# ermongroup/TEOChat

Hardware: AMD Instinct MI355X
Metric: end-to-end tokens/sec (prefill+decode), T=8 frames, LLaMA-2-7B (higher is better)
Workload: dtype bf16; 1 GPU; C3: T=8 frames 224x224 -> CLIP-ViT-L/14 (23 layers) -> mlp2x_gelu -> splice of a 128-token prompt (L=2168) -> LLaMA-2-7B prefill -> 256 forced greedy tokens; value = generated tokens / total time; frames=8, sequence_len=2168, parallelism=dp1 (1 conversation per GPU, no collective), weights=random N(0,0.02^2) at LLaMA-2-7B / ViT-L/14 shapes

## Files before the change

teochat_amd/csrc/gemv.hip:

```cpp
#include <type_traits>

#include "ops.h"
#include "p13.h"

namespace teo {

typedef unsigned char fp8_t;
typedef float f32x2 __attribute__((ext_vector_type(2)));

template <typename T> struct Vec16;
template <> struct Vec16<bf16_t> {
    static constexpr int N = 8;
    __device__ static __forceinline__ void cvt(const uint4& r, float* f) {
        f[0] = __uint_as_float(r.x << 16); f[1] = __uint_as_float(r.x & 0xffff0000u);
        f[2] = __uint_as_float(r.y << 16); f[3] = __uint_as_float(r.y & 0xffff0000u);
        f[4] = __uint_as_float(r.z << 16); f[5] = __uint_as_float(r.z & 0xffff0000u);
        f[6] = __uint_as_float(r.w << 16); f[7] = __uint_as_float(r.w & 0xffff0000u);
    }
};
template <> struct Vec16<f16_t> {
    static constexpr int N = 8;
    __device__ static __forceinline__ void cvt(const uint4& r, float* f) {
        f[0] = h_lo<true>(r.x); f[1] = h_hi<true>(r.x); f[2] = h_lo<true>(r.y); f[3] = h_hi<true>(r.y);
        f[4] = h_lo<true>(r.z); f[5] = h_hi<true>(r.z); f[6] = h_lo<true>(r.w); f[7] = h_hi<true>(r.w);
    }
};
template <> struct Vec16<float> {
    static constexpr int N = 4;
    __device__ static __forceinline__ void cvt(const uint4& r, float* f) {
        f[0] = __uint_as_float(r.x); f[1] = __uint_as_float(r.y); f[2] = __uint_as_float(r.z); f[3] = __uint_as_float(r.w);
    }
};
struct fp4x2_t { unsigned char v; };
template <typename WT> struct IsMx { static constexpr bool v = false; };
template <> struct IsMx<fp4x2_t> { static constexpr bool v = true; };
template <> struct Vec16<fp4x2_t> { static constexpr int N = 32; };
template <typename WT> struct WPer { static constexpr int v = IsMx<WT>::v ? 2 : 1; };
template <typename WT> struct CU { static constexpr int v = Vec16<WT>::N / WPer<WT>::v; };
template <typename WT> using WScaleT = typename std::conditional<IsMx<WT>::v, unsigned char, float>::type;
template <> struct Vec16<fp8_t> {
    static constexpr int N = 16;
    __device__ static __forceinline__ void cvt(const uint4& r, float* f) {
        const unsigned w[4] = {r.x, r.y, r.z, r.w};
#pragma unroll
        for (int i = 0; i < 4; ++i) {
            const f32x2 lo = __builtin_amdgcn_cvt_pk_f32_fp8(w[i], false);
            const f32x2 hi = __builtin_amdgcn_cvt_pk_f32_fp8(w[i], true);
            f[4 * i] = lo.x; f[4 * i + 1] = lo.y; f[4 * i + 2] = hi.x; f[4 * i + 3] = hi.y;
        }
    }
};

template <typename WT>
__device__ __forceinline__ float dot16(const uint4& w, const float* xv, float acc) {
    constexpr int VE = Vec16<WT>::N;
    float f[VE];
    Vec16<WT>::cvt(w, f);
#pragma unroll
    for (int e = 0; e < VE; ++e) acc = fmaf(f[e], xv[e], acc);
    return acc;
}
template <>
__device__ __forceinline__ float dot16<fp8_t>(const uint4& w, const float* xv, float acc) {
    const unsigned ww[4] = {w.x, w.y, w.z, w.w};
#pragma unroll
    for (int i = 0; i < 4; ++i) {
        const f32x2 lo = __builtin_amdgcn_cvt_pk_f32_fp8(ww[i], false);
        const f32x2 hi = __builtin_amdgcn_cvt_pk_f32_fp8(ww[i], true);
        acc = fmaf(lo.x, xv[4 * i], acc);
        acc = fmaf(lo.y, xv[4 * i + 1], acc);
        acc = fmaf(hi.x, xv[4 * i + 2], acc);
        acc = fmaf(hi.y, xv[4 * i + 3], acc);
    }
    return acc;
}

typedef __bf16 gv_bf16x2 __attribute__((ext_vector_type(2)));
__device__ __forceinline__ float dot2bf(unsigned a, unsigned b, float acc) {
    return __builtin_amdgcn_fdot2_f32_bf16(__builtin_bit_cast(gv_bf16x2, a), __builtin_bit_cast(gv_bf16x2, b), acc, false);
}
template <typename WT>
__device__ __forceinline__ float dotb(const uint4& w, const uint4* xv, float acc) {
    constexpr bool F16 = IsF16<WT>::v;
    acc = dot2h<F16>(w.x, xv[0].x, acc); acc = dot2h<F16>(w.y, xv[0].y, acc);
    acc = dot2h<F16>(w.z, xv[0].z, acc); acc = dot2h<F16>(w.w, xv[0].w, acc);
    return acc;
}
template <>
__device__ __forceinline__ float dotb<fp8_t>(const uint4& w, const uint4* xv, float acc) {
    const unsigned ww[4] = {w.x, w.y, w.z, w.w};
    const unsigned xx[8] = {xv[0].x, xv[0].y, xv[0].z, xv[0].w, xv[1].x, xv[1].y, xv[1].z, xv[1].w};
#pragma unroll
    for (int i = 0; i < 4; ++i) {
        const unsigned lo = __builtin_bit_cast(unsigned, __builtin_amdgcn_cvt_scalef32_pk_bf16_fp8(ww[i], 1.0f, false));
        const unsigned hi = __builtin_bit_cast(unsigned, __builtin_amdgcn_cvt_scalef32_pk_bf16_fp8(ww[i], 1.0f, true));
        acc = dot2bf(lo, xx[2 * i], acc);
        acc = dot2bf(hi, xx[2 * i + 1], acc);
    }
    return acc;
}
__device__ __forceinline__ float dot_mx(const uint4& w, const uint4* xv, float escale, float acc) {
    const unsigned ww[4] = {w.x, w.y, w.z, w.w};
#pragma unroll
    for (int i = 0; i < 4; ++i) {
        acc = dot2bf(__builtin_bit_cast(unsigned, __builtin_amdgcn_cvt_scalef32_pk_bf16_fp4(ww[i], escale, 0)), xv[i].x, acc);
        acc = dot2bf(__builtin_bit_cast(unsigned, __builtin_amdgcn_cvt_scalef32_pk_bf16_fp4(ww[i], escale, 1)), xv[i].y, acc);
        acc = dot2bf(__builtin_bit_cast(unsigned, __builtin_amdgcn_cvt_scalef32_pk_bf16_fp4(ww[i], escale, 2)), xv[i].z, acc);
        acc = dot2bf(__builtin_bit_cast(unsigned, __builtin_amdgcn_cvt_scalef32_pk_bf16_fp4(ww[i], escale, 3)), xv[i].w, acc);
    }
    return acc;
}
__device__ __forceinline__ float e8m0_scale(unsigned e) { return __uint_as_float(e << 23); }
template <typename T> struct IsBf { static constexpr bool v = false; };
template <> struct IsBf<bf16_t> { static constexpr bool v = true; };
template <typename T> struct Is16 { static constexpr bool v = IsBf<T>::v || IsF16<T>::v; };
template <typename T, typename WT> struct BfImage { static constexpr bool v = IsBf<T>::v && sizeof(WT) == 1; };
template <typename T, typename WT> struct RowsImage16 { static constexpr bool v = BfImage<T, WT>::v || (IsF16<T>::v && IsF16<WT>::v); };

struct p13_t { unsigned short v; };
template <typename WT> struct IsP13 { static constexpr bool v = false; };
template <> struct IsP13<p13_t> { static constexpr bool v = true; };
template <> struct Vec16<p13_t> {
    static constexpr int N = 8;
    __device__ static __forceinline__ void cvt(const uint4& r, float* f) {
#pragma unroll
        for (int i = 0; i < 4; ++i) { f[i] = __uint_as_float(p13_f32(r.z, r.x, i)); f[4 + i] = __uint_as_float(p13_f32(r.w, r.y, i)); }
    }
};
struct P13Img {
    const unsigned* rt; const unsigned char *lo, *nib, *sgn; const bf16_t* esc;
};
__device__ __forceinline__ P13Img p13_img(const void* W, int N, int K) {
    const P13Layout l = p13_layout(N, K);
    const unsigned char* b = reinterpret_cast<const unsigned char*>(W);
    return {reinterpret_cast<const unsigned*>(b + l.rt), b + l.lo, b + l.nib, b + l.sgn, reinterpret_cast<const bf16_t*>(b + l.esc)};
}
template <bool NT, typename V>
__device__ __forceinline__ V ldv(const void* p) {
    return NT ? __builtin_nontemporal_load(reinterpret_cast<const V*>(p)) : *reinterpret_cast<const V*>(p);
}
template <bool NT>
__device__ __forceinline__ uint4 p13_load(const unsigned char* lo, const unsigned char* nib, const unsigned char* sgn, long long c) {
    typedef unsigned v2u __attribute__((ext_vector_type(2)));
    const v2u l = ldv<NT, v2u>(lo + c * 8);
    return make_uint4(l.x, l.y, ldv<NT, unsigned>(nib + c * 4), (unsigned)ldv<NT, unsigned char>(sgn + c));
}
template <bool PAIRS>
__device__ __forceinline__ uint4 p13_chunk(const uint4& raw, unsigned rpm) {
    if constexpr (PAIRS) {
        unsigned o[4];
        p13_rebuild(raw.x, raw.y, raw.z, raw.w, rpm, o);
        return make_uint4(o[0], o[1], o[2], o[3]);
    } else {
        unsigned h0, h1;
        p13_high(raw.z, raw.w, rpm, h0, h1);
        return make_uint4(raw.x, raw.y, h0, h1);
    }
}
__device__ __forceinline__ unsigned p13_rpm(unsigned rt) { return ((rt & 0xffu) - 1u) * 0x00010001u; }
__device__ __forceinline__ bool p13_escaped(unsigned rt) { return (rt & 0xffu) == 0xffu; }

template <bool NT>
__device__ __forceinline__ uint4 ld16(const void* p) {
    typedef unsigned v4u __attribute__((ext_vector_type(4)));
    const v4u v = NT ? __builtin_nontemporal_load(reinterpret_cast<const v4u*>(p)) : *reinterpret_cast<const v4u*>(p);
    return make_uint4(v.x, v.y, v.z, v.w);
}


template <int VE>
__device__ __forceinline__ int xs_off(int k) {
    const int c = k / VE, g = (k % VE) >> 2;
    return (((c >> 6) * (VE / 4) + g) << 8) + ((c & 63) << 2);
}
template <int VE>
__device__ __forceinline__ int xb_off(int k) {
    const int c = k / VE, g = (k % VE) >> 3;
    return ((((c >> 6) * (VE / 8) + g) << 6) + (c & 63)) * 8 + (k & 7);
}
template <bool XB, int VE>
__device__ __forceinline__ float* x_image_end(float* xs, int nchunk) {
    const int padded = ((nchunk + 63) / 64) * 64 * VE;
    return XB ? reinterpret_cast<float*>(reinterpret_cast<bf16_t*>(xs) + padded) : xs + padded;
}

template <typename T, int VE, bool XB, int XPT, typename F>
__device__ __forceinline__ void stage_x(const T* __restrict__ x, const T* __restrict__ norm_w, float* xs, float* red, int K,
                                        float eps, F after_loads) {
    constexpr int VX = Vec16<T>::N;
    const int tid = threadIdx.x;
    const int nx = K / VX;
    float ss = 0.f;
    if (nx <= XPT * GV_THREADS) {
        uint4 xr[XPT], nr[XPT];
#pragma unroll
        for (int i = 0; i < XPT; ++i) {
            const int c = tid + i * GV_THREADS;
            xr[i] = (c < nx) ? *reinterpret_cast<const uint4*>(x + (long long)c * VX) : make_uint4(0, 0, 0, 0);
        }
        if (norm_w) {
#pragma unroll
            for (int i = 0; i < XPT; ++i) {
                const int c = tid + i * GV_THREADS;
                nr[i] = (c < nx) ? *reinterpret_cast<const uint4*>(norm_w + (long long)c * VX) : make_uint4(0, 0, 0, 0);
            }
        }
        after_loads();
#pragma unroll
        for (int i = 0; i < XPT; ++i) {
            float f[VX];
            Vec16<T>::cvt(xr[i], f);
#pragma unroll
            for (int e = 0; e < VX; ++e) ss = fmaf(f[e], f[e], ss);
        }
        float rr = 1.f;
        if (norm_w) rr = rsqrtf(block_sum<GV_THREADS>(ss, red) / K + eps);
#pragma unroll
        for (int i = 0; i < XPT; ++i) {
            const int c = tid + i * GV_THREADS;
            if (c < nx) {
                float f[VX], g[VX];
                Vec16<T>::cvt(xr[i], f);
                if (norm_w) {
                    Vec16<T>::cvt(nr[i], g);
#pragma unroll
                    for (int e = 0; e < VX; ++e) f[e] = Elem<T>::round(f[e] * rr * g[e]);
                }
                if constexpr (XB) {
                    uint4 o = xr[i];
                    if (norm_w) o = make_uint4(pack_h2<IsF16<T>::v>(f[0], f[1]), pack_h2<IsF16<T>::v>(f[2], f[3]), pack_h2<IsF16<T>::v>(f[4], f[5]),
                                               pack_h2<IsF16<T>::v>(f[6], f[7]));
                    *reinterpret_cast<uint4*>(reinterpret_cast<bf16_t*>(xs) + xb_off<VE>(c * VX)) = o;
                } else {
#pragma unroll
                    for (int e = 0; e < VX; e += 4)
                        *reinterpret_cast<float4*>(xs + xs_off<VE>(c * VX + e)) = make_float4(f[e], f[e + 1], f[e + 2], f[e + 3]);
                }
            }
        }
    } else {
        after_loads();
        for (int c = tid; c < nx; c += GV_THREADS) {
            const uint4 raw = *reinterpret_cast<const uint4*>(x + (long long)c * VX);
            float f[VX];
            Vec16<T>::cvt(raw, f);
#pragma unroll
            for (int e = 0; e < VX; ++e) ss = fmaf(f[e], f[e], ss);
            if constexpr (XB) {
                *reinterpret_cast<uint4*>(reinterpret_cast<bf16_t*>(xs) + xb_off<VE>(c * VX)) = raw;
            } else {
#pragma unroll
                for (int e = 0; e < VX; e += 4)
                    *reinterpret_cast<float4*>(xs + xs_off<VE>(c * VX + e)) = make_float4(f[e], f[e + 1], f[e + 2], f[e + 3]);
            }
        }
        if (norm_w) {
            const float rr = rsqrtf(block_sum<GV_THREADS>(ss, red) / K + eps);
            for (int c = tid; c < nx; c += GV_THREADS) {
                float f[VX];
                Vec16<T>::cvt(*reinterpret_cast<const uint4*>(norm_w + (long long)c * VX), f);
                if constexpr (XB) {
                    uint4* p4 = reinterpret_cast<uint4*>(reinterpret_cast<bf16_t*>(xs) + xb_off<VE>(c * VX));
                    float v[VX];
                    Vec16<T>::cvt(*p4, v);
#pragma unroll
                    for (int e = 0; e < VX; ++e) v[e] = v[e] * rr * f[e];
                    *p4 = make_uint4(pack_h2<IsF16<T>::v>(v[0], v[1]), pack_h2<IsF16<T>::v>(v[2], v[3]), pack_h2<IsF16<T>::v>(v[4], v[5]),
                                     pack_h2<IsF16<T>::v>(v[6], v[7]));
                } else {
#pragma unroll
                    for (int e = 0; e < VX; e += 4) {
                        float4* p4 = reinterpret_cast<float4*>(xs + xs_off<VE>(c * VX + e));
                        float4 v = *p4;
                        v.x = Elem<T>::round(v.x * rr * f[e]); v.y = Elem<T>::round(v.y * rr * f[e + 1]);
                        v.z = Elem<T>::round(v.z * rr * f[e + 2]); v.w = Elem<T>::round(v.w * rr * f[e + 3]);
                        *p4 = v;
                    }
                }
            }
        }
    }
    __syncthreads();
}

template <typename WT, int R, int U, bool NT, bool FULL>
__device__ __forceinline__ void issue_block(uint4 (&w)[U][R], unsigned (&sx)[U][R], const WT* const (&rowp)[R],
                                            const unsigned char* const (&srow)[R], const unsigned char* const (&grow)[R], int c0, int lane,
                                            int nchunk) {
    constexpr int CH = CU<WT>::v;
    if constexpr (IsP13<WT>::v) {
#pragma unroll
        for (int u = 0; u < U; ++u) {
            const int c = c0 + u * 64 + lane;
#pragma unroll
            for (int r = 0; r < R; ++r) {
                if (FULL) w[u][r] = p13_load<NT>(reinterpret_cast<const unsigned char*>(rowp[r]), srow[r], grow[r], c);
                else w[u][r] = (c < nchunk) ? p13_load<NT>(reinterpret_cast<const unsigned char*>(rowp[r]), srow[r], grow[r], c) : make_uint4(0, 0, 0, 0);
            }
        }
        return;
    }
    if constexpr (IsMx<WT>::v) {
#pragma unroll
        for (int u = 0; u < U; ++u) {
            const int c = c0 + u * 64 + lane;
#pragma unroll
            for (int r = 0; r < R; ++r) sx[u][r] = (FULL || c < nchunk) ? (unsigned)srow[r][c] : 0u;
        }
    }
#pragma unroll
    for (int u = 0; u < U; ++u) {
        const int c = c0 + u * 64 + lane;
#pragma unroll
        for (int r = 0; r < R; ++r) {
            if (FULL) w[u][r] = ld16<NT>(rowp[r] + (long long)c * CH);
            else w[u][r] = (c < nchunk) ? ld16<NT>(rowp[r] + (long long)c * CH) : make_uint4(0, 0, 0, 0);
        }
    }
}
template <typename WT, int R, int U, bool PAIRS = false>
__device__ __forceinline__ void rebuild_block(uint4 (&w)[U][R], const unsigned (&rpm)[R]) {
    if constexpr (IsP13<WT>::v) {
#pragma unroll
        for (int u = 0; u < U; ++u)
#pragma unroll
            for (int r = 0; r < R; ++r) w[u][r] = p13_chunk<PAIRS>(w[u][r], rpm[r]);
    }
}
template <typename T, typename WT, int R, int U, bool FULL, bool XB16 = BfImage<T, WT>::v>
__device__ __forceinline__ void consume_block(const uint4 (&w)[U][R], const unsigned (&sx)[U][R], const float* xs, int c0, int lane,
                                              int nchunk, float (&acc)[R]) {
    constexpr int VE = Vec16<WT>::N;
    if constexpr (XB16) {
        float part[U][R];
#pragma unroll
        for (int u = 0; u < U; ++u) {
            const int c = c0 + u * 64 + lane;
            uint4 xb[VE / 8];
#pragma unroll
            for (int j = 0; j < VE / 8; ++j)
                xb[j] = (FULL || c < nchunk) ? *reinterpret_cast<const uint4*>(reinterpret_cast<const bf16_t*>(xs) + xb_off<VE>(c * VE + j * 8))
                                             : make_uint4(0, 0, 0, 0);
#pragma unroll
            for (int r = 0; r < R; ++r) {
                if constexpr (IsMx<WT>::v) part[u][r] = dot_mx(w[u][r], xb, e8m0_scale(sx[u][r]), 0.f);
                else part[u][r] = dotb<WT>(w[u][r], xb, 0.f);
            }
        }
#pragma unroll
        for (int r = 0; r < R; ++r) {
            float t = part[0][r];
#pragma unroll
            for (int u = 1; u < U; ++u) t += part[u][r];
            acc[r] += t;
        }
        return;
    } else {
#pragma unroll
    for (int u = 0; u < U; ++u) {
        const int c = c0 + u * 64 + lane;
        float xv[VE];
        if (FULL || c < nchunk) {
#pragma unroll
            for (int e = 0; e < VE; e += 4) {
                const float4 t = *reinterpret_cast<const float4*>(xs + xs_off<VE>(c * VE + e));
                xv[e] = t.x; xv[e + 1] = t.y; xv[e + 2] = t.z; xv[e + 3] = t.w;
            }
        } else {
#pragma unroll
            for (int e = 0; e < VE; ++e) xv[e] = 0.f;
        }
#pragma unroll
        for (int r = 0; r < R; ++r) acc[r] = dot16<WT>(w[u][r], xv, acc[r]);
        if (VE > 8) __builtin_amdgcn_sched_barrier(0);
    }
    }
}

template <typename T, int U, bool NT, bool XB16>
__device__ __forceinline__ float rows_escaped_row(const bf16_t* row, const float* xs, int lane, int nchunk) {
    constexpr int STEP = 64 * U;
    const bf16_t* rowp[1] = {row};
    const unsigned char* none[1] = {nullptr};
    uint4 w[U][1];
    unsigned sx[U][1];
    float acc[1] = {0.f};
    const int cfull = (nchunk / STEP) * STEP;
    int c0 = 0;
    for (; c0 < cfull; c0 += STEP) {
        issue_block<bf16_t, 1, U, NT, true>(w, sx, rowp, none, none, c0, lane, nchunk);
        consume_block<T, bf16_t, 1, U, true, XB16>(w, sx, xs, c0, lane, nchunk, acc);
    }
    if (c0 < nchunk) {
        issue_block<bf16_t, 1, U, NT, false>(w, sx, rowp, none, none, c0, lane, nchunk);
        consume_block<T, bf16_t, 1, U, false, XB16>(w, sx, xs, c0, lane, nchunk, acc);
    }
    return acc[0];
}

template <typename T, typename TO, typename WT, int R, int U, bool PF, bool NT, bool SWIGLU, int XPT>
__global__ __launch_bounds__(GV_THREADS) void gemv_kernel(const T* __restrict__ x, const WT* __restrict__ W,
                                                          const WScaleT<WT>* __restrict__ wscale, const T* __restrict__ norm_w,
                                                          const T* res, TO* y, int N, int K,
                                                          float eps) {
    extern __shared__ __attribute__((aligned(16))) float xs[];
    constexpr int VE = Vec16<WT>::N;
    constexpr int STEP = 64 * U;
    const int lane = threadIdx.x & 63, wid = threadIdx.x >> 6;
    const int nchunk = K / VE;
    float* red = x_image_end<RowsImage16<T, WT>::v, VE>(xs, nchunk);
    const int nwaves = gridDim.x * GV_WAVES;
    const int ngroups = SWIGLU ? (N / 2 + (R / 2) - 1) / (R / 2) : (N + R - 1) / R;

    auto row_of = [&](int grp, int r) -> long long {
        if (SWIGLU) {
            const int j = min(grp * (R / 2) + (r >> 1), N / 2 - 1);
            return (long long)((j >> 4) * 32 + (j & 15) + ((r & 1) ? 16 : 0));
        }
        return (long long)min(grp * R + r, N - 1);
    };

    uint4 wa[U][R];
    unsigned sa[U][R];
    const long long rowlen = K / WPer<WT>::v;
    P13Img img = {};
    if constexpr (IsP13<WT>::v) img = p13_img(W, N, K);
    auto row_ptrs = [&](long long row, const WT*& wp, const unsigned char*& sp, const unsigned char*& gp) {
        if constexpr (IsP13<WT>::v) {
            wp = reinterpret_cast<const WT*>(img.lo + row * K); sp = img.nib + row * (K / 2); gp = img.sgn + row * (K / 8);
        } else {
            wp = W + row * rowlen;
            sp = IsMx<WT>::v ? reinterpret_cast<const unsigned char*>(wscale) + row * nchunk : nullptr;
            gp = nullptr;
        }
    };
    int grp = blockIdx.x * GV_WAVES + wid;
    stage_x<T, VE, RowsImage16<T, WT>::v, XPT>(x, norm_w, xs, red, K, eps, [&]() {
        if (PF) {
            const int gp = min(grp, ngroups - 1);
            const WT* rowp[R];
            const unsigned char *srow[R], *grow[R];
#pragma unroll
            for (int r = 0; r < R; ++r) row_ptrs(row_of(gp, r), rowp[r], srow[r], grow[r]);
            issue_block<WT, R, U, NT, true>(wa, sa, rowp, srow, grow, 0, lane, nchunk);
        }
    });

    bool have = PF;
    for (; grp < ngroups; grp += nwaves) {
        const WT* rowp[R];
        const unsigned char *srow[R], *grow[R];
        long long rows[R];
#pragma unroll
        for (int r = 0; r < R; ++r) {
            rows[r] = row_of(grp, r);
            row_ptrs(rows[r], rowp[r], srow[r], grow[r]);
        }
        float sc[R];
#pragma unroll
        for (int r = 0; r < R; ++r) sc[r] = (!IsMx<WT>::v && !IsP13<WT>::v && wscale) ? (float)wscale[rows[r]] : 1.f;
        unsigned rt[R], rpm[R];
#pragma unroll
        for (int r = 0; r < R; ++r) { rt[r] = IsP13<WT>::v ? img.rt[rows[r]] : 0u; rpm[r] = p13_rpm(rt[r]); }
        float acc[R];
#pragma unroll
        for (int r = 0; r < R; ++r) acc[r] = 0.f;
        int c0 = 0;
        if (have) {
            rebuild_block<WT, R, U>(wa, rpm);
            consume_block<T, WT, R, U, true, RowsImage16<T, WT>::v>(wa, sa, xs, 0, lane, nchunk, acc); c0 = STEP; have = false;
        }
        const int cfull = (nchunk / STEP) * STEP;
        for (; c0 < cfull; c0 += STEP) {
            issue_block<WT, R, U, NT, true>(wa, sa, rowp, srow, grow, c0, lane, nchunk);
            rebuild_block<WT, R, U>(wa, rpm);
            consume_block<T, WT, R, U, true, RowsImage16<T, WT>::v>(wa, sa, xs, c0, lane, nchunk, acc);
        }
        if (c0 < nchunk) {
            issue_block<WT, R, U, NT, false>(wa, sa, rowp, srow, grow, c0, lane, nchunk);
            rebuild_block<WT, R, U>(wa, rpm);
            consume_block<T, WT, R, U, false, RowsImage16<T, WT>::v>(wa, sa, xs, c0, lane, nchunk, acc);
        }
        if constexpr (IsP13<WT>::v) {
#pragma unroll
            for (int r = 0; r < R; ++r)
                if (p13_escaped(rt[r]))
                    acc[r] = rows_escaped_row<T, U, NT, RowsImage16<T, WT>::v>(img.esc + (long long)(rt[r] >> 8) * K, xs, lane, nchunk);
        }
#pragma unroll
        for (int r = 0; r < R; ++r) acc[r] = wave_sum(acc[r]);
        if (lane == 0) {
#pragma unroll
            for (int r = 0; r < R; ++r) acc[r] *= sc[r];
            if (SWIGLU) {
#pragma unroll
                for (int p = 0; p < R / 2; ++p) {
                    const int j = grp * (R / 2) + p;
                    if (j < N / 2) Elem<TO>::st(y + j, silu(acc[2 * p]) * acc[2 * p + 1]);
                }
            } else {
#pragma unroll
                for (int r = 0; r < R; ++r) {
                    const int n = grp * R + r;
                    if (n < N) {
                        float v = acc[r];
                        if (res) v += Elem<T>::ld(res + n);
                        Elem<TO>::st(y + n, v);
                    }
                }
            }
        }
    }
}

template <typename T, typename TO, typename WT, int R, int U, bool NT>
__global__ __launch_bounds__(GV_THREADS) void gemv_splitk_kernel(const T* __restrict__ x, const WT* __restrict__ W,
                                                                 const WScaleT<WT>* __restrict__ wscale, const T* res,
                                                                 TO* y, int N, int K) {
    constexpr int VE = Vec16<WT>::N, VX = Vec16<T>::N;
    constexpr int XL = VE / VX;
    __shared__ float part[GV_WAVES][R];
    const int tid = threadIdx.x, lane = tid & 63, wid = tid >> 6;
    const int nchunk = K / VE;
    const int row0 = blockIdx.x * R;
    const float my_scale = (!IsMx<WT>::v && !IsP13<WT>::v && wscale && tid < R && row0 + tid < N) ? (float)wscale[row0 + tid] : 1.f;
    const float my_res = (res && tid < R && row0 + tid < N) ? Elem<T>::ld(res + row0 + tid) : 0.f;
    float acc[R];
#pragma unroll
    for (int r = 0; r < R; ++r) acc[r] = 0.f;
    const WT* wrow[R];
    const unsigned char* srow[R];
    const unsigned char* grow[R];
    unsigned rt[R], rpm[R];
    P13Img img = {};
    if constexpr (IsP13<WT>::v) img = p13_img(W, N, K);
#pragma unroll
    for (int r = 0; r < R; ++r) {
        const long long row = min(row0 + r, N - 1);
        if constexpr (IsP13<WT>::v) {
            wrow[r] = reinterpret_cast<const WT*>(img.lo + row * K); srow[r] = img.nib + row * (K / 2); grow[r] = img.sgn + row * (K / 8);
            rt[r] = img.rt[row];
        } else {
            wrow[r] = W + row * (K / WPer<WT>::v);
            srow[r] = IsMx<WT>::v ? reinterpret_cast<const unsigned char*>(wscale) + row * nchunk : nullptr;
            grow[r] = nullptr; rt[r] = 0u;
        }
        rpm[r] = p13_rpm(rt[r]);
    }
    auto step = [&](int cb, auto full_tag) {
        constexpr bool FULL = decltype(full_tag)::value;
        uint4 xr[U][XL];
        uint4 w[U][R];
        unsigned sx[U][R];
        if constexpr (IsMx<WT>::v) {
#pragma unroll
            for (int u = 0; u < U; ++u) {
                const int c = cb + u * 256 + wid * 64 + lane;
#pragma unroll
                for (int r = 0; r < R; ++r) sx[u][r] = (FULL || c < nchunk) ? (unsigned)srow[r][c] : 0u;
            }
        }
#pragma unroll
        for (int u = 0; u < U; ++u) {
            const int c = cb + u * 256 + wid * 64 + lane;
#pragma unroll
            for (int j = 0; j < XL; ++j)
                xr[u][j] = (FULL || c < nchunk) ? *reinterpret_cast<const uint4*>(x + (long long)c * VE + j * VX) : make_uint4(0, 0, 0, 0);
        }
#pragma unroll
        for (int u = 0; u < U; ++u) {
            const int c = cb + u * 256 + wid * 64 + lane;
#pragma unroll
            for (int r = 0; r < R; ++r) {
                if constexpr (IsP13<WT>::v)
                    w[u][r] = (FULL || c < nchunk) ? p13_load<NT>(reinterpret_cast<const unsigned char*>(wrow[r]), srow[r], grow[r], c) : make_uint4(0, 0, 0, 0);
                else
                    w[u][r] = (FULL || c < nchunk) ? ld16<NT>(wrow[r] + (long long)c * CU<WT>::v) : make_uint4(0, 0, 0, 0);
            }
        }
        rebuild_block<WT, R, U, true>(w, rpm);
#pragma unroll
        for (int u = 0; u < U; ++u) {
            if constexpr (IsMx<WT>::v) {
#pragma unroll
                for (int r = 0; r < R; ++r) acc[r] = dot_mx(w[u][r], xr[u], e8m0_scale(sx[u][r]), acc[r]);
            } else if constexpr (Is16<T>::v) {
#pragma unroll
                for (int r = 0; r < R; ++r) acc[r] = dotb<WT>(w[u][r], xr[u], acc[r]);
            } else {
                float xv[VE];
#pragma unroll
                for (int j = 0; j < XL; ++j) Vec16<T>::cvt(xr[u][j], xv + j * VX);
#pragma unroll
                for (int r = 0; r < R; ++r) acc[r] = dot16<WT>(w[u][r], xv, acc[r]);
            }
        }
    };
    const int cfull = (nchunk / (256 * U)) * (256 * U);
    int cb = 0;
    for (; cb < cfull; cb += 256 * U) step(cb, std::true_type{});
    for (; cb < nchunk; cb += 256 * U) step(cb, std::false_type{});
    if constexpr (IsP13<WT>::v) {
#pragma unroll
        for (int r = 0; r < R; ++r) {
            if (p13_escaped(rt[r])) {
                const bf16_t* raw = img.esc + (long long)(rt[r] >> 8) * K;
                float a = 0.f;
                auto estep = [&](int cb2, auto full_tag) {
                    constexpr bool FULL = decltype(full_tag)::value;
                    uint4 xr[U], w[U];
#pragma unroll
                    for (int u = 0; u < U; ++u) {
                        const int c = cb2 + u * 256 + wid * 64 + lane;
                        xr[u] = (FULL || c < nchunk) ? *reinterpret_cast<const uint4*>(x + (long long)c * VE) : make_uint4(0, 0, 0, 0);
                    }
#pragma unroll
                    for (int u = 0; u < U; ++u) {
                        const int c = cb2 + u * 256 + wid * 64 + lane;
                        w[u] = (FULL || c < nchunk) ? ld16<NT>(raw + (long long)c * VE) : make_uint4(0, 0, 0, 0);
                    }
#pragma unroll
                    for (int u = 0; u < U; ++u) a = dotb<bf16_t>(w[u], &xr[u], a);
                };
                int c2 = 0;
                for (; c2 < cfull; c2 += 256 * U) estep(c2, std::true_type{});
                for (; c2 < nchunk; c2 += 256 * U) estep(c2, std::false_type{});
                acc[r] = a;
            }
        }
    }
#pragma unroll
    for (int r = 0; r < R; ++r) acc[r] = wave_sum(acc[r]);
    if (lane == 0) {
#pragma unroll
        for (int r = 0; r < R; ++r) part[wid][r] = acc[r];
    }
    __syncthreads();
    if (tid < R) {
        const int n = row0 + tid;
        if (n < N) {
            float v = (part[0][tid] + part[1][tid]) + (part[2][tid] + part[3][tid]);
            v *= my_scale;
            v += my_res;
            Elem<TO>::st(y + n, v);
        }
    }
}

template <typename T, typename WT, bool NT, bool PF, int U, int XPT>
__global__ __launch_bounds__(GV_THREADS) void gemv_qkv_rope_kernel(const WT* __restrict__ W, const T* __restrict__ x,
                                                                   const T* __restrict__ norm_w, const WScaleT<WT>* __restrict__ wscale,
                                                                   const int* __restrict__ d_pos, int K, int H, int Hk, int hd,
                                                                   T* __restrict__ qout, const float* __restrict__ cs,
                                                                   const float* __restrict__ sn, T* __restrict__ kc,
                                                                   T* __restrict__ vc, T* __restrict__ vtc, int S_max, float eps) {
    extern __shared__ __attribute__((aligned(16))) float xs[];
    constexpr int VE = Vec16<WT>::N;
    constexpr int R = 2, STEP = 64 * U;
    const int lane = threadIdx.x & 63, wid = threadIdx.x >> 6;
    const int nchunk = K / VE;
    float* red = x_image_end<BfImage<T, WT>::v, VE>(xs, nchunk);
    const int half = hd >> 1, half_log2 = __builtin_ctz((unsigned)hd) - 1;
    const int qk_groups = (H + Hk) * half;
    const int ngroups = qk_groups + (Hk * hd) / 2;
    const int nwaves = gridDim.x * GV_WAVES;
    const int pos = *d_pos;

    auto rows_of = [&](int grp, long long (&rows)[R], int& head, int& i0) -> bool {
        const bool qk = grp < qk_groups;
        if (qk) {
            head = grp >> half_log2;
            i0 = grp & (half - 1);
            rows[0] = (long long)head * hd + i0;
            rows[1] = rows[0] + half;
        } else {
            rows[0] = (long long)(H + Hk) * hd + (grp - qk_groups) * 2;
            rows[1] = rows[0] + 1;
        }
        return qk;
    };

    uint4 wa[U][R];
    unsigned sa[U][R];
    const long long rowlen = K / WPer<WT>::v;
    const unsigned char* sbase = IsMx<WT>::v ? reinterpret_cast<const unsigned char*>(wscale) : nullptr;
    P13Img img = {};
    if constexpr (IsP13<WT>::v) img = p13_img(W, (H + 2 * Hk) * hd, K);
    auto row_ptrs = [&](long long row, const WT*& wp, const unsigned char*& sp, const unsigned char*& gp) {
        if constexpr (IsP13<WT>::v) {
            wp = reinterpret_cast<const WT*>(img.lo + row * K); sp = img.nib + row * (K / 2); gp = img.sgn + row * (K / 8);
        } else {
            wp = W + row * rowlen; sp = sbase ? sbase + row * nchunk : nullptr; gp = nullptr;
        }
    };
    const int grp0 = blockIdx.x * GV_WAVES + wid;
    stage_x<T, VE, BfImage<T, WT>::v, XPT>(x, norm_w, xs, red, K, eps, [&]() {
        if (PF) {
            long long rows[R];
            int head, i0;
            rows_of(min(grp0, ngroups - 1), rows, head, i0);
            const WT* rowp[R];
            const unsigned char *srow[R], *grow[R];
#pragma unroll
            for (int r = 0; r < R; ++r) row_ptrs(rows[r], rowp[r], srow[r], grow[r]);
            issue_block<WT, R, U, NT, true>(wa, sa, rowp, srow, grow, 0, lane, nchunk);
        }
    });

    bool have = PF;
    for (int grp = grp0; grp < ngroups; grp += nwaves) {
        long long rows[R];
        int head = 0, i0 = 0;
        const bool is_qk = rows_of(grp, rows, head, i0);
        const WT* rowp[R];
        const unsigned char *srow[R], *grow[R];
#pragma unroll
        for (int r = 0; r < R; ++r) row_ptrs(rows[r], rowp[r], srow[r], grow[r]);
        float rc = 1.f, rs = 0.f;
        if (is_qk) { rc = cs[(long long)pos * half + i0]; rs = sn[(long long)pos * half + i0]; }
        constexpr bool SCALED = !IsMx<WT>::v && !IsP13<WT>::v;
        const float sc0 = (SCALED && wscale) ? (float)wscale[rows[0]] : 1.f, sc1 = (SCALED && wscale) ? (float)wscale[rows[1]] : 1.f;
        unsigned rt[R], rpm[R];
#pragma unroll
        for (int r = 0; r < R; ++r) { rt[r] = IsP13<WT>::v ? img.rt[rows[r]] : 0u; rpm[r] = p13_rpm(rt[r]); }
        float acc[R] = {0.f, 0.f};
        int c0 = 0;
        if (have) {
            rebuild_block<WT, R, U>(wa, rpm);
            consume_block<T, WT, R, U, true>(wa, sa, xs, 0, lane, nchunk, acc); c0 = STEP; have = false;
        }
        const int cfull = (nchunk / STEP) * STEP;
        for (; c0 < cfull; c0 += STEP) {
            issue_block<WT, R, U, NT, true>(wa, sa, rowp, srow, grow, c0, lane, nchunk);
            rebuild_block<WT, R, U>(wa, rpm);
            consume_block<T, WT, R, U, true>(wa, sa, xs, c0, lane, nchunk, acc);
        }
        if (c0 < nchunk) {
            issue_block<WT, R, U, NT, false>(wa, sa, rowp, srow, grow, c0, lane, nchunk);
            rebuild_block<WT, R, U>(wa, rpm);
            consume_block<T, WT, R, U, false>(wa, sa, xs, c0, lane, nchunk, acc);
        }
        if constexpr (IsP13<WT>::v) {
#pragma unroll
            for (int r = 0; r < R; ++r)
                if (p13_escaped(rt[r]))
                    acc[r] = rows_escaped_row<T, U, NT, BfImage<T, WT>::v>(img.esc + (long long)(rt[r] >> 8) * K, xs, lane, nchunk);
        }
#pragma unroll
        for (int r = 0; r < R; ++r) acc[r] = wave_sum(acc[r]);
        if (lane == 0) {
            acc[0] *= sc0; acc[1] *= sc1;
            if (is_qk) {
                const float x1 = Elem<T>::round(acc[0]), x2 = Elem<T>::round(acc[1]);
                const float y1 = x1 * rc - x2 * rs, y2 = x2 * rc + x1 * rs;
                if (head < H) {
                    Elem<T>::st(qout + head * hd + i0, y1);
                    Elem<T>::st(qout + head * hd + i0 + half, y2);
                } else {
                    T* dst = kc + ((long long)(head - H) * S_max + pos) * hd;
                    Elem<T>::st(dst + i0, y1);
                    Elem<T>::st(dst + i0 + half, y2);
                }
            } else {
                const int v0 = (grp - qk_groups) * 2;
#pragma unroll
                for (int r = 0; r < R; ++r) {
                    const int hk = (v0 + r) >> (half_log2 + 1), d = (v0 + r) & (hd - 1);
                    T val;
                    Elem<T>::st(&val, acc[r]);
                    vc[((long long)hk * S_max + pos) * hd + d] = val;
                    if (vtc) vtc[((long long)hk * hd + d) * S_max + pos] = val;
                }
            }
        }
    }
}

struct GemvArgs {
    const void *x, *W, *ws, *norm_w, *res;
    void* y;
    int N, K;
    float eps;
};

template <typename T, typename TO, typename WT, int R, int U, bool PF, int XPT>
static int rows_form(const GemvPlan& g, const GemvArgs& a, hipStream_t st) {
    with_flags([&](auto nt, auto sw) {
        TEO_KLAUNCH((gemv_kernel<T, TO, WT, R, U, PF, decltype(nt)::value, decltype(sw)::value, XPT>), g.blocks, GV_THREADS, g.lds_bytes, st,
                    (const T*)a.x, (const WT*)a.W, (const WScaleT<WT>*)a.ws, (const T*)a.norm_w, (const T*)a.res, (TO*)a.y, a.N, a.K, a.eps);
    }, g.nt, g.swiglu);
    TEO_LAUNCH_CHECK("gemv");
    return TEO_OK;
}
template <typename T, typename TO, typename WT>
static int launch_rows(const GemvPlan& g, const GemvArgs& a, hipStream_t st) {
#define TEO_GV_FORM(R_, U_, PF_, XPT_) \
    if (g.R == R_ && g.U == U_ && g.prefetch == PF_ && g.xpt == XPT_) return rows_form<T, TO, WT, R_, U_, PF_, XPT_>(g, a, st)
    TEO_GV_FORM(4, 2, false, 6); TEO_GV_FORM(2, 4, false, 6); TEO_GV_FORM(2, 8, true, 6); TEO_GV_FORM(2, 8, false, 6);
    if constexpr (sizeof(WT) == 1) {
        TEO_GV_FORM(2, 4, true, 2); TEO_GV_FORM(4, 2, true, 2); TEO_GV_FORM(2, 2, true, 2); TEO_GV_FORM(4, 4, true, 2);
        TEO_GV_FORM(2, 4, true, 6); TEO_GV_FORM(4, 2, true, 6); TEO_GV_FORM(2, 2, true, 6); TEO_GV_FORM(4, 4, true, 6);
        TEO_GV_FORM(2, 2, false, 6); TEO_GV_FORM(4, 4, false, 6);
    } else if constexpr (IsP13<WT>::v) {
        TEO_GV_FORM(2, 4, false, 2);
        TEO_GV_FORM(2, 4, true, 2); TEO_GV_FORM(2, 4, true, 6);
    } else {
        TEO_GV_FORM(2, 4, true, 6);
        if constexpr (Is16<T>::v) TEO_GV_FORM(2, 4, true, 2);
    }
#undef TEO_GV_FORM
    set_error("gemv: no row kernel of %d x %d, prefetch %d, %d x chunks for this weight format", g.R, g.U, (int)g.prefetch, g.xpt);
    return TEO_ERR_UNSUPPORTED;
}

template <typename T, typename TO, typename WT, int R, int U>
static int splitk_form(const GemvPlan& g, const GemvArgs& a, hipStream_t st) {
    with_flags([&](auto nt) {
        TEO_KLAUNCH((gemv_splitk_kernel<T, TO, WT, R, U, decltype(nt)::value>), g.blocks, GV_THREADS, 0, st, (const T*)a.x, (const WT*)a.W,
                    (const WScaleT<WT>*)a.ws, (const T*)a.res, (TO*)a.y, a.N, a.K);
    }, g.nt);
    TEO_LAUNCH_CHECK("gemv_splitk");
    return TEO_OK;
}
template <typename T, typename TO, typename WT>
static int launch_splitk(const GemvPlan& g, const GemvArgs& a, hipStream_t st) {
    switch (g.R * 10 + g.U) {
        case 21: return splitk_form<T, TO, WT, 2, 1>(g, a, st);
        case 22: return splitk_form<T, TO, WT, 2, 2>(g, a, st);
        case 23: return splitk_form<T, TO, WT, 2, 3>(g, a, st);
        case 24: return splitk_form<T, TO, WT, 2, 4>(g, a, st);
        case 26: return splitk_form<T, TO, WT, 2, 6>(g, a, st);
        case 41: return splitk_form<T, TO, WT, 4, 1>(g, a, st);
        case 42: return splitk_form<T, TO, WT, 4, 2>(g, a, st);
        case 43: return splitk_form<T, TO, WT, 4, 3>(g, a, st);
        case 44: return splitk_form<T, TO, WT, 4, 4>(g, a, st);
        case 46: return splitk_form<T, TO, WT, 4, 6>(g, a, st);
        default: break;
    }
    set_error("gemv: no split-K kernel of %d rows x %d chunks", g.R, g.U);
    return TEO_ERR_UNSUPPORTED;
}

template <typename T, typename TO, typename WT>
static int gemv_launch(const GemvPlan& g, const GemvArgs& a, hipStream_t st) {
    return g.kind == GemvKind::SplitK ? launch_splitk<T, TO, WT>(g, a, st) : launch_rows<T, TO, WT>(g, a, st);
}

int gemv_w(const void* x, const void* W, const void* wscale, int wfmt, const void* norm_w, const void* res, void* y, int N,
           int K, float eps, unsigned flags, int dtype, int out_dtype, hipStream_t st, GemvPlan* plan_only) {
    if (N == 0) return TEO_OK;
    const bool swiglu = flags & TEO_GEMM_SWIGLU16;
    const bool w_fp8 = wfmt == GV_W_FP8, w_mx = wfmt == GV_W_MXFP4, w_p13 = wfmt == GV_W_P13;
    if (w_p13) {
        TEO_CHECK_ARG(dtype == TEO_BF16, "teo_gemv: a w13 image holds bf16 weights and needs bf16 activations (dtype %d)", dtype);
        if (K % 8 != 0) {
            set_error("teo_gemv: K=%d is not a multiple of the w13 image's 8-element chunk", K);
            return TEO_ERR_UNSUPPORTED;
        }
    }
    const int ve = w_mx ? 32 : (w_fp8 ? 16 : (dtype == TEO_F32 ? 4 : 8));
    TEO_CHECK_ARG(K % ve == 0, "teo_gemv: K=%d must be a multiple of %d", K, ve);
    TEO_CHECK_ARG((reinterpret_cast<uintptr_t>(W) & 15) == 0, "teo_gemv: W must be 16-byte aligned");
    TEO_CHECK_ARG((size_t)(K + 1040) * 4 <= 64 * 1024, "teo_gemv: K=%d too large for LDS staging", K);
    TEO_CHECK_ARG((reinterpret_cast<uintptr_t>(x) & 15) == 0 && (norm_w == nullptr || (reinterpret_cast<uintptr_t>(norm_w) & 15) == 0),
                  "teo_gemv: x / norm_w must be 16-byte aligned");
    if (swiglu) TEO_CHECK_ARG(N % 32 == 0 && !res, "teo_gemv: SWIGLU16 needs N %% 32 == 0 and no residual");
    if (w_mx) TEO_CHECK_ARG(dtype == TEO_BF16 && wscale != nullptr, "teo_gemv: MXFP4 weights need bf16 activations and block scales");
    else if (w_fp8) TEO_CHECK_ARG(dtype == TEO_BF16 && wscale != nullptr, "teo_gemv: fp8 weights need bf16 activations and per-row scales");
    else if (!w_p13 && dtype == TEO_F32) TEO_CHECK_ARG(out_dtype == TEO_F32, "teo_gemv: f32 inputs need f32 output");
    else if (!w_p13 && dtype != TEO_BF16 && dtype != TEO_F16) {
        set_error("teo_gemv: unknown dtype %d", dtype);
        return TEO_ERR_UNSUPPORTED;
    }
    const GemvPlan g = plan_gemv({N, K, wfmt, dtype, out_dtype, swiglu, norm_w != nullptr, 0, 0, 0}, tune());
    if (plan_only) { *plan_only = g; return TEO_OK; }
    const GemvArgs a = {x, W, (w_fp8 || w_mx) ? wscale : nullptr, norm_w, res, y, N, K, eps};
    const bool of32 = out_dtype == TEO_F32;
    if (w_mx) return of32 ? gemv_launch<bf16_t, float, fp4x2_t>(g, a, st) : gemv_launch<bf16_t, bf16_t, fp4x2_t>(g, a, st);
    if (w_p13) return of32 ? gemv_launch<bf16_t, float, p13_t>(g, a, st) : gemv_launch<bf16_t, bf16_t, p13_t>(g, a, st);
    if (w_fp8) return of32 ? gemv_launch<bf16_t, float, fp8_t>(g, a, st) : gemv_launch<bf16_t, bf16_t, fp8_t>(g, a, st);
    if (dtype == TEO_F32) return gemv_launch<float, float, float>(g, a, st);
    if (dtype == TEO_BF16) return of32 ? gemv_launch<bf16_t, float, bf16_t>(g, a, st) : gemv_launch<bf16_t, bf16_t, bf16_t>(g, a, st);
    return of32 ? gemv_launch<f16_t, float, f16_t>(g, a, st) : gemv_launch<f16_t, f16_t, f16_t>(g, a, st);
}

int gemv(const void* x, const void* W, const void* norm_w, const void* res, void* y, int N, int K, float eps,
         unsigned flags, int dtype, int out_dtype, hipStream_t st) {
    return gemv_w(x, W, nullptr, GV_W_NATIVE, norm_w, res, y, N, K, eps, flags, dtype, out_dtype, st);
}

struct QkvArgs {
    const void *x, *W, *ws, *norm_w;
    void* qout;
    const float *cs, *sn;
    const int* d_pos;
    void *kc, *vc, *vtc;
    int S_max, H, Hk, hd, K;
    float eps;
};
template <typename T, typename WT, int U, int XPT>
static int qkv_form(const GemvPlan& g, const QkvArgs& a, hipStream_t st) {
    with_flags([&](auto nt, auto pf) {
        TEO_KLAUNCH((gemv_qkv_rope_kernel<T, WT, decltype(nt)::value, decltype(pf)::value, U, XPT>), g.blocks, GV_THREADS, g.lds_bytes, st,
                    (const WT*)a.W, (const T*)a.x, (const T*)a.norm_w, (const WScaleT<WT>*)a.ws, a.d_pos, a.K, a.H, a.Hk, a.hd, (T*)a.qout, a.cs,
                    a.sn, (T*)a.kc, (T*)a.vc, (T*)a.vtc, a.S_max, a.eps);
    }, g.nt, g.prefetch);
    TEO_LAUNCH_CHECK("gemv_qkv_rope");
    return TEO_OK;
}
template <typename T, typename WT>
static int launch_qkv(const GemvPlan& g, const QkvArgs& a, hipStream_t st) {
    if constexpr (IsMx<WT>::v) {
        if (g.U == 2 && g.xpt == 2) return qkv_form<T, WT, 2, 2>(g, a, st);
        if (g.U == 2 && g.xpt == 6) return qkv_form<T, WT, 2, 6>(g, a, st);
    } else {
        if constexpr (Is16<T>::v) { if (g.U == 4 && g.xpt == 2) return qkv_form<T, WT, 4, 2>(g, a, st); }
        if (g.U == 4 && g.xpt == 6) return qkv_form<T, WT, 4, 6>(g, a, st);
        if constexpr (sizeof(WT) == 1) { if (g.U == 2 && g.xpt == 6) return qkv_form<T, WT, 2, 6>(g, a, st); }
    }
    set_error("gemv_qkv_rope: no kernel of %d chunks per step, %d x chunks for this weight format", g.U, g.xpt);
    return TEO_ERR_UNSUPPORTED;
}

int gemv_qkv_rope(const void* x, const void* W, const void* wscale, int wfmt, const void* norm_w, void* qout,
                  const float* cs, const float* sn, const int* d_pos, void* kc, void* vc, void* vtc, int S_max, int H, int Hk,
                  int hd, int K, float eps, int dtype, hipStream_t st, GemvPlan* plan_only) {
    const bool w_fp8 = wfmt == GV_W_FP8, w_mx = wfmt == GV_W_MXFP4, w_p13 = wfmt == GV_W_P13;
    TEO_CHECK_ARG(!w_p13 || dtype == TEO_BF16, "gemv_qkv_rope: a w13 image needs bf16 activations");
    const int ve = w_mx ? 32 : (w_fp8 ? 16 : (dtype == TEO_F32 ? 4 : 8));
    TEO_CHECK_ARG(K % ve == 0 && hd >= 2 && (hd & (hd - 1)) == 0, "gemv_qkv_rope: K=%d hd=%d (head_dim must be a power of two)", K, hd);
    TEO_CHECK_ARG((size_t)(K + 1040) * 4 <= 64 * 1024, "gemv_qkv_rope: K=%d too large for LDS staging", K);
    TEO_CHECK_ARG(!(w_fp8 || w_mx) || (dtype == TEO_BF16 && wscale), "gemv_qkv_rope: fp8 / MXFP4 weights need bf16 activations and scales");
    const GemvPlan g = plan_gemv_qkv({(H + 2 * Hk) * hd, K, wfmt, dtype, dtype, false, norm_w != nullptr, H, Hk, hd}, tune());
    if (plan_only) { *plan_only = g; return TEO_OK; }
    const QkvArgs a = {x, W, wscale, norm_w, qout, cs, sn, d_pos, kc, vc, vtc, S_max, H, Hk, hd, K, eps};
    if (w_mx) return launch_qkv<bf16_t, fp4x2_t>(g, a, st);
    if (w_fp8) return launch_qkv<bf16_t, fp8_t>(g, a, st);
    if (w_p13) return launch_qkv<bf16_t, p13_t>(g, a, st);
    if (dtype == TEO_F32) return launch_qkv<float, float>(g, a, st);
    if (dtype == TEO_F16) return launch_qkv<f16_t, f16_t>(g, a, st);
    return launch_qkv<bf16_t, bf16_t>(g, a, st);
}

}
```

Before: 383.2 tokens/s.

## Add double-buffered ring streaming for P13 weight GEMV and QKV-RoPE kernels

For P13-compressed weights, the GEMV and fused QKV+RoPE kernels gain a ring-buffered streaming path. It issues the next row-group's weight block, or the next row's first block, while consuming the current one. Each wave walks its row groups continuously, so no latency bubble appears at row boundaries. The path also sets waves-per-EU occupancy hints for this configuration and double-buffers the x/weight loads in the row-per-block loop. It raises register pressure and code complexity, and needs nchunk to be a multiple of the step.

```diff
diff --git a/teochat_amd/csrc/gemv.hip b/teochat_amd/csrc/gemv.hip
--- a/teochat_amd/csrc/gemv.hip
+++ b/teochat_amd/csrc/gemv.hip
@@ -398,8 +398,114 @@
     return acc[0];
 }
 
+template <typename WT, int R, int U> struct P13RingWaves { static constexpr int v = (IsP13<WT>::v && R == 2 && U == 4) ? 4 : 0; };
+template <int R> struct P13Rows { const unsigned char *lo[R], *nib[R], *sgn[R]; };
+template <int R, int U, bool NT>
+__device__ __forceinline__ void p13_issue_full(uint4 (&w)[U][R], const P13Rows<R>& b, unsigned lane) {
+    typedef unsigned v2u __attribute__((ext_vector_type(2)));
+    asm volatile("" : "+v"(lane));
+    lane &= 63u;
+#pragma unroll
+    for (int u = 0; u < U; ++u) {
+#pragma unroll
+        for (int r = 0; r < R; ++r) {
+            const v2u l = ldv<NT, v2u>(b.lo[r] + (lane * 8u + u * 512u));
+            w[u][r] = make_uint4(l.x, l.y, ldv<NT, unsigned>(b.nib[r] + (lane * 4u + u * 256u)),
+                                 (unsigned)ldv<NT, unsigned char>(b.sgn[r] + (lane + u * 64u)));
+        }
+    }
+}
+template <int R>
+__device__ __forceinline__ P13Rows<R> p13_rows_at(const P13Img& img, const long long (&rows)[R], int K, int c0) {
+    P13Rows<R> b;
+#pragma unroll
+    for (int r = 0; r < R; ++r) {
+        b.lo[r] = img.lo + rows[r] * K + (long long)c0 * 8;
+        b.nib[r] = img.nib + rows[r] * (K / 2) + (long long)c0 * 4;
+        b.sgn[r] = img.sgn + rows[r] * (K / 8) + c0;
+    }
+    return b;
+}
+template <int R, int U, bool NT, typename RowsOf>
+__device__ __forceinline__ void p13_ring_issue(uint4 (&w)[U][R], unsigned (&rtn)[R], const P13Img& img, int K, int g, int c0, unsigned lane,
+                                               RowsOf rows_of) {
+    long long rows[R];
+    rows_of(g, rows);
+#pragma unroll
+    for (int r = 0; r < R; ++r) rtn[r] = img.rt[rows[r]];
+    p13_issue_full<R, U, NT>(w, p13_rows_at<R>(img, rows, K, c0), lane);
+}
+template <int R, int U>
+__device__ __forceinline__ void p13_consume(const uint4 (&w)[U][R], const unsigned (&rpm)[R], const float* xs, int c0, int lane, float (&acc)[R]) {
+    constexpr int VE = Vec16<p13_t>::N;
+    float xv[2][VE];
+    const float* xl = xs + (((unsigned)c0 >> 6) * (VE / 4) << 8) + ((unsigned)lane << 2);
+    auto read_x = [&](int u) {
+#pragma unroll
+        for (int e = 0; e < VE; e += 4) {
+            const float4 t = *reinterpret_cast<const float4*>(xl + ((u * (VE / 4) + (e >> 2)) << 8));
+            xv[u & 1][e] = t.x; xv[u & 1][e + 1] = t.y; xv[u & 1][e + 2] = t.z; xv[u & 1][e + 3] = t.w;
+        }
+    };
+    read_x(0);
+#pragma unroll
+    for (int u = 0; u < U; ++u) {
+        if (u + 1 < U) read_x(u + 1);
+#pragma unroll
+        for (int r = 0; r < R; ++r) acc[r] = dot16<p13_t>(p13_chunk<false>(w[u][r], rpm[r]), xv[u & 1], acc[r]);
+        __builtin_amdgcn_sched_barrier(0);
+    }
+}
+template <typename T, int R, int U, bool NT, bool XB16, typename RowsOf, typename Begin, typename Store>
+__device__ __forceinline__ void p13_rows_stream(uint4 (&s0)[U][R], uint4 (&s1)[U][R], unsigned (&rtn)[R], const P13Img& img, int K, int nchunk,
+                                                const float* xs, int lane, int grp, int nwaves, int ngroups, RowsOf rows_of, Begin begin,
+                                                Store store) {
+    static_assert(!XB16, "bf16 weights meet the fp32 x image");
+    constexpr int STEP = 64 * U;
+    const int nfull = nchunk / STEP;
+    if (grp >= ngroups) return;
+    unsigned rt[R], rpm[R];
+    float acc[R];
+    int blk = 0;
+    auto open = [&]() {
+#pragma unroll
+        for (int r = 0; r < R; ++r) { rt[r] = rtn[r]; rpm[r] = p13_rpm(rt[r]); acc[r] = 0.f; }
+        begin(grp);
+    };
+    auto close = [&]() {
+        int ln = lane;
+        asm volatile("" : "+v"(ln));
+#pragma unroll
+        for (int r = 0; r < R; ++r)
+            if (p13_escaped(rt[r])) acc[r] = rows_escaped_row<T, U, NT, XB16>(img.esc + (long long)(rt[r] >> 8) * K, xs, ln, nchunk);
+#pragma unroll
+        for (int r = 0; r < R; ++r) acc[r] = wave_sum(acc[r]);
+        store(grp, acc);
+    };
+    auto turn = [&](uint4 (&a)[U][R], uint4 (&b)[U][R]) {
+        const bool last = blk + 1 == nfull;
+        p13_ring_issue<R, U, NT>(b, rtn, img, K, last ? min(grp + nwaves, ngroups - 1) : grp, last ? 0 : (blk + 1) * STEP, lane, rows_of);
+        __builtin_amdgcn_sched_barrier(0);
+        p13_consume<R, U>(a, rpm, xs, blk * STEP, lane, acc);
+        if (last) {
+            close();
+            grp += nwaves, blk = 0;
+            if (grp < ngroups) open();
+        } else {
+            ++blk;
+        }
+    };
+    open();
+    for (;;) {
+        turn(s0, s1);
+        if (grp >= ngroups) break;
+        turn(s1, s0);
+        if (grp >= ngroups) break;
+    }
+}
+
 template <typename T, typename TO, typename WT, int R, int U, bool PF, bool NT, bool SWIGLU, int XPT>
-__global__ __launch_bounds__(GV_THREADS) void gemv_kernel(const T* __restrict__ x, const WT* __restrict__ W,
+__global__ __launch_bounds__(GV_THREADS) __attribute__((amdgpu_waves_per_eu(P13RingWaves<WT, R, U>::v))) void gemv_kernel(const T* __restrict__ x, const WT* __restrict__ W,
                                                           const WScaleT<WT>* __restrict__ wscale, const T* __restrict__ norm_w,
                                                           const T* res, TO* y, int N, int K,
                                                           float eps) {
@@ -434,6 +540,40 @@
             gp = nullptr;
         }
     };
+    if constexpr (IsP13<WT>::v) if (nchunk > 0 && nchunk % STEP == 0) {
+        const int grp0 = blockIdx.x * GV_WAVES + __builtin_amdgcn_readfirstlane(wid);
+        uint4 wb[U][R];
+        unsigned rtn[R];
+        auto rows_of = [&](int g, long long (&rows)[R]) {
+#pragma unroll
+            for (int r = 0; r < R; ++r) rows[r] = row_of(g, r);
+        };
+        stage_x<T, VE, RowsImage16<T, WT>::v, XPT>(x, norm_w, xs, red, K, eps, [&]() {
+            p13_ring_issue<R, U, NT>(wa, rtn, img, K, min(grp0, ngroups - 1), 0, lane, rows_of);
+        });
+        p13_rows_stream<T, R, U, NT, RowsImage16<T, WT>::v>(wa, wb, rtn, img, K, nchunk, xs, lane, grp0, nwaves, ngroups, rows_of, [](int) {},
+                                                            [&](int g, float (&acc)[R]) {
+            if (lane != 0) return;
+            if (SWIGLU) {
+#pragma unroll
+                for (int p = 0; p < R / 2; ++p) {
+                    const int j = g * (R / 2) + p;
+                    if (j < N / 2) Elem<TO>::st(y + j, silu(acc[2 * p]) * acc[2 * p + 1]);
+                }
+            } else {
+#pragma unroll
+                for (int r = 0; r < R; ++r) {
+                    const int n = g * R + r;
+                    if (n < N) {
+                        float v = acc[r];
+                        if (res) v += Elem<T>::ld(res + n);
+                        Elem<TO>::st(y + n, v);
+                    }
+                }
+            }
+        });
+        return;
+    }
     int grp = blockIdx.x * GV_WAVES + wid;
     stage_x<T, VE, RowsImage16<T, WT>::v, XPT>(x, norm_w, xs, red, K, eps, [&]() {
         if (PF) {
@@ -571,14 +711,9 @@
         for (int u = 0; u < U; ++u) {
             const int c = cb + u * 256 + wid * 64 + lane;
 #pragma unroll
-            for (int r = 0; r < R; ++r) {
-                if constexpr (IsP13<WT>::v)
-                    w[u][r] = (FULL || c < nchunk) ? p13_load<NT>(reinterpret_cast<const unsigned char*>(wrow[r]), srow[r], grow[r], c) : make_uint4(0, 0, 0, 0);
-                else
-                    w[u][r] = (FULL || c < nchunk) ? ld16<NT>(wrow[r] + (long long)c * CU<WT>::v) : make_uint4(0, 0, 0, 0);
-            }
-        }
-        rebuild_block<WT, R, U, true>(w, rpm);
+            for (int r = 0; r < R; ++r)
+                w[u][r] = (FULL || c < nchunk) ? ld16<NT>(wrow[r] + (long long)c * CU<WT>::v) : make_uint4(0, 0, 0, 0);
+        }
 #pragma unroll
         for (int u = 0; u < U; ++u) {
             if constexpr (IsMx<WT>::v) {
@@ -597,9 +732,78 @@
         }
     };
     const int cfull = (nchunk / (256 * U)) * (256 * U);
-    int cb = 0;
-    for (; cb < cfull; cb += 256 * U) step(cb, std::true_type{});
-    for (; cb < nchunk; cb += 256 * U) step(cb, std::false_type{});
+    if constexpr (IsP13<WT>::v) {
+        constexpr int STEP = 256 * U;
+        const int wv = __builtin_amdgcn_readfirstlane(wid);
+        const unsigned char* xb = reinterpret_cast<const unsigned char*>(x) + wv * (64 * 16);
+        P13Rows<R> base;
+#pragma unroll
+        for (int r = 0; r < R; ++r) {
+            base.lo[r] = reinterpret_cast<const unsigned char*>(wrow[r]) + wv * (64 * 8); base.nib[r] = srow[r] + wv * (64 * 4); base.sgn[r] = grow[r] + wv * 64;
+        }
+        auto issue = [&](uint4 (&xr)[U], uint4 (&w)[U][R], int cb, auto full_tag) {
+            constexpr bool FULL = decltype(full_tag)::value;
+            typedef unsigned v2u __attribute__((ext_vector_type(2)));
+            const unsigned char* xp = xb + (long long)cb * 16;
+            unsigned ln = lane;
+            asm volatile("" : "+v"(ln));
+            ln &= 63u;
+#pragma unroll
+            for (int u = 0; u < U; ++u) {
+                const int c = cb + u * 256 + wv * 64 + lane;
+                xr[u] = (FULL || c < nchunk) ? *reinterpret_cast<const uint4*>(xp + (ln * 16u + u * 4096u)) : make_uint4(0, 0, 0, 0);
+            }
+#pragma unroll
+            for (int u = 0; u < U; ++u) {
+                const int c = cb + u * 256 + wv * 64 + lane;
+#pragma unroll
+                for (int r = 0; r < R; ++r) {
+                    if (FULL || c < nchunk) {
+                        const v2u l = ldv<NT, v2u>(base.lo[r] + (long long)cb * 8 + (ln * 8u + u * 2048u));
+                        w[u][r] = make_uint4(l.x, l.y, ldv<NT, unsigned>(base.nib[r] + (long long)cb * 4 + (ln * 4u + u * 1024u)),
+                                             (unsigned)ldv<NT, unsigned char>(base.sgn[r] + cb + (ln + u * 256u)));
+                    } else {
+                        w[u][r] = make_uint4(0, 0, 0, 0);
+                    }
+                }
+            }
+        };
+        auto compute = [&](const uint4 (&xr)[U], uint4 (&w)[U][R]) {
+            rebuild_block<WT, R, U, true>(w, rpm);
+#pragma unroll
+            for (int u = 0; u < U; ++u) {
+#pragma unroll
+                for (int r = 0; r < R; ++r) acc[r] = dotb<WT>(w[u][r], &xr[u], acc[r]);
+            }
+        };
+        uint4 x0[U], x1[U], w0[U][R], w1[U][R];
+        int cb = 0;
+        auto turn = [&](uint4 (&xa)[U], uint4 (&wa)[U][R], uint4 (&xn)[U], uint4 (&wn)[U][R]) {
+            const int nx = cb + STEP;
+            if (nx < cfull) issue(xn, wn, nx, std::true_type{});
+            else if (nx < nchunk) issue(xn, wn, nx, std::false_type{});
+            compute(xa, wa);
+            cb = nx;
+        };
+        if (cfull > 0) issue(x0, w0, 0, std::true_type{});
+        else if (nchunk > 0) issue(x0, w0, 0, std::false_type{});
+        bool in1 = false;
+        while (cb < cfull) {
+            turn(x0, w0, x1, w1);
+            in1 = true;
+            if (cb >= cfull) break;
+            turn(x1, w1, x0, w0);
+            in1 = false;
+        }
+        if (cb < nchunk) {
+            if (in1) compute(x1, w1);
+            else compute(x0, w0);
+        }
+    } else {
+        int cb = 0;
+        for (; cb < cfull; cb += 256 * U) step(cb, std::true_type{});
+        for (; cb < nchunk; cb += 256 * U) step(cb, std::false_type{});
+    }
     if constexpr (IsP13<WT>::v) {
 #pragma unroll
         for (int r = 0; r < R; ++r) {
@@ -648,7 +852,7 @@
 }
 
 template <typename T, typename WT, bool NT, bool PF, int U, int XPT>
-__global__ __launch_bounds__(GV_THREADS) void gemv_qkv_rope_kernel(const WT* __restrict__ W, const T* __restrict__ x,
+__global__ __launch_bounds__(GV_THREADS) __attribute__((amdgpu_waves_per_eu(P13RingWaves<WT, 2, U>::v))) void gemv_qkv_rope_kernel(const WT* __restrict__ W, const T* __restrict__ x,
                                                                    const T* __restrict__ norm_w, const WScaleT<WT>* __restrict__ wscale,
                                                                    const int* __restrict__ d_pos, int K, int H, int Hk, int hd,
                                                                    T* __restrict__ qout, const float* __restrict__ cs,
@@ -693,9 +897,57 @@
             wp = W + row * rowlen; sp = sbase ? sbase + row * nchunk : nullptr; gp = nullptr;
         }
     };
+    if constexpr (IsP13<WT>::v) if (nchunk > 0 && nchunk % STEP == 0) {
+        const int g0 = blockIdx.x * GV_WAVES + __builtin_amdgcn_readfirstlane(wid);
+        uint4 wb[U][R];
+        unsigned rtn[R];
+        auto rows_only = [&](int g, long long (&rows)[R]) {
+            int head, i0;
+            rows_of(g, rows, head, i0);
+        };
+        stage_x<T, VE, BfImage<T, WT>::v, XPT>(x, norm_w, xs, red, K, eps, [&]() {
+            p13_ring_issue<R, U, NT>(wa, rtn, img, K, min(g0, ngroups - 1), 0, lane, rows_only);
+        });
+        bool is_qk = false;
+        int head = 0, i0 = 0;
+        float rc = 1.f, rs = 0.f;
+        p13_rows_stream<T, R, U, NT, BfImage<T, WT>::v>(wa, wb, rtn, img, K, nchunk, xs, lane, g0, nwaves, ngroups, rows_only,
+                                                        [&](int g) {
+            long long rows[R];
+            is_qk = rows_of(g, rows, head, i0);
+            rc = 1.f, rs = 0.f;
+            if (is_qk) { rc = cs[(long long)pos * half + i0]; rs = sn[(long long)pos * half + i0]; }
+        },
+                                                        [&](int g, float (&acc)[R]) {
+            if (lane != 0) return;
+            if (is_qk) {
+                const float x1 = Elem<T>::round(acc[0]), x2 = Elem<T>::round(acc[1]);
+                const float y1 = x1 * rc - x2 * rs, y2 = x2 * rc + x1 * rs;
+                if (head < H) {
+                    Elem<T>::st(qout + head * hd + i0, y1);
+                    Elem<T>::st(qout + head * hd + i0 + half, y2);
+                } else {
+                    T* dst = kc + ((long long)(head - H) * S_max + pos) * hd;
+                    Elem<T>::st(dst + i0, y1);
+                    Elem<T>::st(dst + i0 + half, y2);
+                }
+            } else {
+                const int v0 = (g - qk_groups) * 2;
+#pragma unroll
+                for (int r = 0; r < R; ++r) {
+                    const int hk = (v0 + r) >> (half_log2 + 1), d = (v0 + r) & (hd - 1);
+                    T val;
+                    Elem<T>::st(&val, acc[r]);
+                    vc[((long long)hk * S_max + pos) * hd + d] = val;
+                    if (vtc) vtc[((long long)hk * hd + d) * S_max + pos] = val;
+                }
+            }
+        });
+        return;
+    }
     const int grp0 = blockIdx.x * GV_WAVES + wid;
     stage_x<T, VE, BfImage<T, WT>::v, XPT>(x, norm_w, xs, red, K, eps, [&]() {
-        if (PF) {
+        if (PF && !IsP13<WT>::v) {
             long long rows[R];
             int head, i0;
             rows_of(min(grp0, ngroups - 1), rows, head, i0);
@@ -707,7 +959,7 @@
         }
     });
 
-    bool have = PF;
+    bool have = PF && !IsP13<WT>::v;
     for (int grp = grp0; grp < ngroups; grp += nwaves) {
         long long rows[R];
         int head = 0, i0 = 0;
```

Result: slower. 372.9 tokens/s (-2.7%).
